# waiwera/waiwera

Measured on AMD Instinct MI355X. Metric: Newton steps/sec, 10M-cell eos_we (BCSR SpMV GB/s in roofline), higher is better.
Workload: dtype f64

## Files before the change

waiwera_amd/csrc/context.hpp:

```cpp
#pragma once
#include <hip/hip_runtime.h>
#include <string>
#include <type_traits>
#include <vector>
#include "../../include/waiwera_hip.h"
#include "devbuf.hpp"
#include "physics.hip.h"

namespace wai {

__host__ __device__ __forceinline__ size_t ell_ld(size_t n) {
  size_t ld = (n + 511) & ~(size_t)511;
  if ((ld & 262143) == 0) ld += 512;
  return ld;
}
__host__ __device__ __forceinline__ size_t ell_rows(int bs, size_t n) {
  if (bs >= 3) return ell_ld(n);
  return n;
}
__host__ __device__ __forceinline__ size_t ell_ix1(int bs, size_t n, int r, int k, size_t i) {
  if (bs >= 3) return ((i >> 6) * (size_t)(bs * bs) + (size_t)(r * bs + k)) * 64 + (i & 63);
  return ((size_t)r * n + i) * bs + k;
}
__host__ __device__ __forceinline__ size_t ell_ix(int bs, size_t n, int s, int r, int k, size_t i) {
// ... 40 lines not shown
  DevBuf<int> cell_src;
  DevBuf<int> face_cells;
};

struct Sources {
  int n = 0;
  DevBuf<int> cell, comp, next;
  DevBuf<double> rate, enth;
  DevBuf<SrcCtl> ctl;
  DevBuf<double> net;
};

struct NetNode { double rate = 0, enth = 0, wrate = 0, wenth = 0, srate = 0, senth = 0; };
struct NetRef { int kind = 0, index = -1; };
struct NetGroup {
  std::vector<NetRef> in;
  int scaling = 0;
  int n_limit = 0, limit_type[3] = {0, 0, 0};
  double limit[3] = {0, 0, 0};
  SrcCtl sep{};
  NetNode node;
};
struct NetOutput {
  int flow = 1;
  NetRef out;
  double rate = -1.0, proportion = -1.0, enthalpy = -1.0;
  NetNode node;
};
struct NetReinjector {
  NetRef in;
  std::vector<NetOutput> out;
  NetRef overflow;
  NetNode node;
  double in_w = 0, in_wh = 0, in_s = 0, in_sh = 0;
  double out_w = 0, out_s = 0;
  NetNode over;
  bool fed = false;
};
struct Network {
  bool on = false;
  std::vector<NetGroup> groups;
  std::vector<NetReinjector> reinjectors;
  std::vector<int> reinj_order;
  std::vector<int> rate_specified, enth_specified;
  std::vector<NetNode> src;
  std::vector<double> h_enth0, h_raw, out_rate, out_enth;
  std::vector<char> is_out;
  std::vector<SrcCtl> h_ctl;
  DevBuf<double> d_raw;
  std::vector<int> gidx;
  int n_global = 0;
  DevBuf<double> d_all;
  std::vector<double> h_loc, l_net, l_enth;
  std::vector<int> h_cell;
  bool coupling = true;
  bool cp_in_pc = true;
  bool cp_valid = false;
  std::vector<int> cp_cells;
  std::vector<double> h_cp_val;
  bool cp_span = false;
  int cp_m = 0, cp_j0 = 0;
  std::vector<int> cp_owner;
  DevBuf<int> d_cp_cells;
  DevBuf<double> d_cp_val, d_cp_f, d_cp_g;
  DevBuf<double> d_cp_x;
};

struct Bcsr {
  int n = 0, ncols = 0, nnzb = 0, bs = 0, W = 0;
  int* col = nullptr;
  double* val = nullptr;
  int* rowptr = nullptr;
  int dg = 0;
  double* fdg = nullptr;
};
struct Pattern {
  int n = 0, ncols = 0, nnzb = 0, W = 0;
  DevBuf<int> col;
  DevBuf<int> rowptr;
  std::vector<int> h_rowptr, h_colidx;
};

struct LinSys;
struct IluSchedule {
  int nsub = 0, max_rows = 0, max_lev = 0;
  DevBuf<int> sub_ptr;
  DevBuf<int> sub_nlev;
  DevBuf<int> sub_split;
  DevBuf<int> row_info;
  bool wide = false;
  DevBuf<unsigned long long> row_infow;
  DevBuf<double> fval;
  DevBuf<double> dinv;
  bool diag_only = false;
  bool scaled = true;
  bool park = true;
  DevBuf<int> row_uoff;
  DevBuf<int> row_tslot;
  int max_nl = 0;
  bool park2 = false;
  DevBuf<int> sub_int;
  DevBuf<int> sub_bnd;
  int n_int = 0, n_bnd = 0;
  DevBuf<int> sub_order;
  int max_ublocks = 0;
  bool fast3 = false;
  int max_nlu = 0;
  bool rows_kernel = false;
  bool wave_kernel = false;
  DevBuf<int> row_uoffw;
  int max_ublocks_w = 0;
  DevBuf<unsigned short> col16;
  DevBuf<int> sub_seg;
  bool level_sorted = false;
  bool big = false;
  bool sublu = false;
  int nlev_f = 0, nlev_b = 0;
  DevBuf<int> ord_f;
  DevBuf<int> ord_b;
  std::vector<int> lev_f_ptr, lev_b_ptr;
  bool built = false;
  const LinSys* owner = nullptr;
};
inline int pc_threads(const IluSchedule& s) { return ((s.max_rows + 63) / 64) * 64; }

template <class F>
int with_bs(int bs, F&& f) {
  switch (bs) {
    case 1: f(std::integral_constant<int, 1>{}); return 0;
    case 2: f(std::integral_constant<int, 2>{}); return 0;
    case 3: f(std::integral_constant<int, 3>{}); return 0;
    case 4: f(std::integral_constant<int, 4>{}); return 0;
    default: return -1;
  }
}
template <class F>
void with_flag(bool flag, F&& f) {
  if (flag) f(std::true_type{});
  else f(std::false_type{});
}
template <class F>
int with_eos(int kind, F&& f) {
  switch (kind) {
    case EOS_W: f(std::integral_constant<int, EOS_W>{}); return 0;
    case EOS_WE: f(std::integral_constant<int, EOS_WE>{}); return 0;
    case EOS_WCE: f(std::integral_constant<int, EOS_WCE>{}); return 0;
    case EOS_WSE: f(std::integral_constant<int, EOS_WSE>{}); return 0;
    case EOS_WAE: f(std::integral_constant<int, EOS_WAE>{}); return 0;
    case EOS_WSCE: f(std::integral_constant<int, EOS_WSCE>{}); return 0;
    case EOS_WSAE: f(std::integral_constant<int, EOS_WSAE>{}); return 0;
    default: return -1;
  }
}
struct EosTraits { int np, df, nmob; bool salt; };
inline int eos_traits(int kind, EosTraits& t) {
  return with_eos(kind, [&](auto k) {
    constexpr int K = decltype(k)::value;
    t = EosTraits{EosT<K>::np, EosT<K>::df, EosT<K>::nmob, is_salt<K>};
  });
}

struct AsmSystem {
  int overlap = -1;
  int levels = 0;
  bool sublu = false;
  int n_ext = 0;
  Bcsr E;
  DevBuf<int> E_col;
  DevBuf<double> E_val;
  IluSchedule sched;
  DevBuf<int> ext_row;
  DevBuf<int> gmap;
  DevBuf<double> r_ext;
  bool with_net = false;
  int n_net = 0;
  DevBuf<int> net_pos;
  DevBuf<int> net_pair;
  bool cross = false;
  DevBuf<double> hval;
  DevBuf<double> r_full;
};

struct ResForm {
  int method = 0;
  double dt = 0.0, ratio = 0.0;
  const double* last = nullptr;
  const double* last2 = nullptr;
};

constexpr int MAX_TRACERS = 8;
constexpr int POST_OFF = 64;
constexpr unsigned long long POST_KEY = 0x5bd1e995a5a5c3c3ull;
struct Tracers {
  int nt = 0;
  int phase[MAX_TRACERS] = {0};
  double decay[MAX_TRACERS] = {0}, activation[MAX_TRACERS] = {0}, diffusion[MAX_TRACERS] = {0};
// ... 245 lines not shown
```

waiwera_amd/csrc/kernels_fused.hip:

```cpp
#include "pc_generic.hip.h"
#include "pc_wide.hip.h"
#include "pc_park.hip.h"
#include "pc_rows.hip.h"
#include "pc_wave.hip.h"
#include "krylov_vec.hip.h"

namespace wai {

static inline int vgrid(int n) {
  int g = (n + TPB - 1) / TPB;
  return g > 1024 ? 1024 : (g < 1 ? 1 : g);
}

void read_env(wai_ctx* c) {
  c->env.fin_separate = getenv("WAI_FIN_SEPARATE") != nullptr;
  c->env.no_col16 = getenv("WAI_NO_COL16") != nullptr;
  c->env.scalar_kernels = getenv("WAI_BCGS_SCALAR_KERNELS") != nullptr;
}

int pc_kernel_kind(const wai_ctx* c, const Bcsr& J, const IluSchedule& s) {
  if (J.dg) return -1;
  if (s.wide) return 4;
  if (c->dbg) return 0;
  if (s.wave_kernel && J.bs >= 3) return 3;
  if (s.rows_kernel) return 2;
  if (J.bs == 2 && s.park && s.diag_only && s.scaled && s.fast3 && pc_threads(s) <= 512) return 1;
  return 0;
}
static bool kind_composes(int kind) { return kind >= 1 && kind <= 3; }
bool pc_axpy_capable(const wai_ctx* c, const Bcsr& M) { return !c->ilu.big && kind_composes(pc_kernel_kind(c, M, c->ilu)); }
bool pc_axpy_default(const wai_ctx* c, const Bcsr& M) {
  if (c->ilu.big) return false;
  const int kind = pc_kernel_kind(c, M, c->ilu);
  return (kind == 1 && c->ilu.col16 && !c->env.no_col16) || kind == 3;
}

template <int BS>
static void launch_pc_bs(wai_ctx* c, const Bcsr& J, const IluSchedule& s, bool spmv, const double* in, double* z,
                         int dot_mode, const double* aux, const int* list, int nrun, const Fin* finp, const double* in2) {
  if (!list) { nrun = s.nsub; list = s.sub_order; }
  const bool with_fin = finp && dot_mode != 0;
  Fin fin;
  if (finp && dot_mode != 0) { fin = *finp; fin.count = nrun; fin.nb = s.nsub; fin.nf = fin_slices(s.nsub); }
  c->ks.n_launch++;
  const int grid = ((nrun + 7) / 8) * 8 + (with_fin ? fin.nf : 0), T = pc_threads(s);
  const size_t lds = ((size_t)T * BS + 80) * sizeof(double);
  auto sp_ax = [&](auto&& go) {
    if (spmv) with_flag(in2 != nullptr, [&](auto ax) { go(std::true_type{}, ax); });
    else go(std::false_type{}, std::false_type{});
  };
  const int kind = pc_kernel_kind(c, J, s);
  const double* scal = c->ks.scal;
  const int* rp = (size_t)J.nnzb * 10 < (size_t)J.n * J.W * 9 ? J.rowptr : nullptr;
  if (kind == 4) {
    const size_t room = (size_t)64 * 1024 > lds ? (size_t)64 * 1024 - lds : 0;
    const int ucap = (int)std::min((size_t)s.max_ublocks_w, room / ((size_t)BS * BS * sizeof(double)));
    const size_t lds_w = lds + (size_t)ucap * BS * BS * sizeof(double);
    with_flag(spmv, [&](auto sp) {
      hipLaunchKernelGGL((k_pc_wide<BS, decltype(sp)::value>), grid, T, lds_w, c->stream, J.n, J.W, nrun, s.sub_ptr, s.sub_nlev,
                         s.row_infow, s.row_uoffw, J.col, rp, J.val, s.fval, in, z, aux, c->ks.partials, c->ks.nb_max,
                         dot_mode, ucap, list, fin);
    });
    return;
  }
  if (kind == 3) {
    if constexpr (BS >= 3) {
      const int ngrp = (nrun + 3) / 4;
      const int pbase = (list && list == s.sub_bnd) ? (s.n_int + 3) / 4 : 0, nb_w = pbase + ngrp;
      if (with_fin) { fin.nb = nb_w; fin.nf = fin_slices(nb_w); }
      c->ks.nb_pc = nb_w;
      const int gridw = ((ngrp + 7) / 8) * 8 + (with_fin ? fin.nf : 0);
      const int per = 64 * BS + s.max_ublocks_w * BS * BS;
      const size_t lds_w = (size_t)4 * per * sizeof(double);
      Stagger stagger;
      stagger.ncu = c->n_cu;
      stagger.per_cu = std::max(1, (int)((size_t)160 * 1024 / (lds_w + 864)));
      stagger.ticks = 400;
      sp_ax([&](auto sp, auto ax) {
        hipLaunchKernelGGL((k_pc_wave<BS, decltype(sp)::value, decltype(ax)::value>), gridw, 256, lds_w, c->stream, J.n, J.W, nrun,
                           s.sub_ptr, s.sub_nlev, s.row_info, s.row_uoffw, J.col, s.fval, s.dinv, in, in2, scal, z, aux, c->ks.partials,
                           c->ks.nb_max, dot_mode, list, rp, s.sub_split, per, pbase, fin, stagger);
      });
      return;
    }
  }
  if (kind == 2) {
    const int TR = ((s.max_rows * BS + 63) / 64) * 64;
    const size_t lds_r = ((size_t)s.max_rows * BS + BS + 5 * 16 + 8) * sizeof(double);
    auto rows = [&](auto nlu) {
      sp_ax([&](auto sp, auto ax) {
        constexpr int NLU = decltype(nlu)::value;
        hipLaunchKernelGGL((k_pc_rows<BS, decltype(sp)::value, NLU, NLU, decltype(ax)::value>), grid, TR, lds_r, c->stream, J.n, J.W,
                           nrun, s.sub_ptr, s.sub_nlev, s.row_info, J.col, s.fval, s.dinv, in, in2, scal, z, aux, c->ks.partials,
                           c->ks.nb_max, dot_mode, list, rp, s.sub_split, fin);
      });
    };
    if (s.max_nlu <= 3) rows(std::integral_constant<int, 3>{});
    else rows(std::integral_constant<int, 4>{});
    return;
  }
  if constexpr (BS == 2) {
    if (kind == 1) {
      const size_t lds_park = lds + (size_t)s.max_ublocks * 4 * sizeof(double);
      Stagger stagger;
      stagger.ncu = c->n_cu;
      stagger.per_cu = std::max(1, std::min(3, (int)((size_t)160 * 1024 / (lds_park + 704))));
      stagger.ticks = 600;
      with_flag(s.col16 && !c->env.no_col16, [&](auto c16) {
        sp_ax([&](auto sp, auto ax) {
          hipLaunchKernelGGL((k_pc_park<decltype(sp)::value, decltype(ax)::value, decltype(c16)::value>), grid, T, lds_park, c->stream,
                             J.n, J.W, nrun, s.sub_ptr, s.sub_nlev, s.row_info, s.row_uoff, J.col, s.col16, s.sub_seg, s.fval, s.dinv,
                             in, in2, scal, z, aux, c->ks.partials, c->ks.nb_max, dot_mode, list, fin, stagger);
        });
      });
      return;
    }
  }
  auto generic = [&](auto di) {
    with_flag(spmv, [&](auto sp) {
      with_flag(s.fast3, [&](auto fast) {
        hipLaunchKernelGGL((k_pc<BS, decltype(sp)::value, decltype(di)::value, decltype(fast)::value>), grid, T, lds, c->stream,
                           J.n, J.W, nrun, s.sub_ptr, s.sub_nlev, s.row_info, J.col, J.val, s.fval, s.dinv, in, z, aux,
                           c->ks.partials, c->ks.nb_max, dot_mode, c->dbg, list, fin);
      });
    });
  };
  if (s.diag_only && s.scaled) generic(std::integral_constant<int, 2>{});
  else if (s.diag_only) generic(std::integral_constant<int, 1>{});
  else generic(std::integral_constant<int, 0>{});
}

int launch_pc_on(wai_ctx* c, const Bcsr& M, const IluSchedule& s, bool spmv, const double* in, double* z,
                 int dot_mode, const double* aux, const int* list, int nrun, const Fin* fin, const double* in2) {
  if (in2 && (!spmv || !kind_composes(pc_kernel_kind(c, M, s)))) { c->err = "composed input asked of a kernel that cannot form it"; return -1; }
  const Fin* fin_later = nullptr;
  if (fin && dot_mode != 0 && c->env.fin_separate) { fin_later = fin; fin = nullptr; }
  if (M.dg) {
    c->ks.n_launch++;
    if (launch_dg_pc(c, M, s, spmv, in, z, list, nrun)) return -1;
    if (dot_mode == PC_DOT_NONE) return 0;
    const int n = M.dg * M.n, s0 = pc_dot_slot0(dot_mode);
    if (dot_mode == PC_DOT_ZA || dot_mode == PC_DOT_ZZ) vec_dots(c, z, dot_mode == PC_DOT_ZA ? aux : z, s0, nullptr, nullptr, 0, n);
    else {
      vec_dots(c, in, z, s0, z, z, s0 + 1, n);
      if (dot_mode == PC_DOT_MERGED) { vec_dots(c, in, in, s0 + 2, in, aux, s0 + 3, n); vec_dots(c, z, aux, s0 + 4, nullptr, nullptr, 0, n); }
    }
    if (const Fin* f = fin ? fin : fin_later) {
      if (dot_mode == PC_DOT_MERGED) { vec_finalize(c, c->ks.nb_pc, s0, 4, -1); vec_finalize(c, c->ks.nb_pc, s0 + 4, 1, f->phase); }
      else vec_finalize(c, c->ks.nb_pc, s0, pc_dot_nslots(dot_mode), f->phase);
      if (f->seq > 0) bcgs_post(c, f->seq);
    }
    return 0;
  }
  c->ks.nb_pc = s.nsub;
  if (with_bs(M.bs, [&](auto bs) { launch_pc_bs<decltype(bs)::value>(c, M, s, spmv, in, z, dot_mode, aux, list, nrun, fin, in2); }) != 0)
    return -1;
  if (fin_later) {
    vec_finalize(c, c->ks.nb_pc, fin_later->slot0, fin_later->nslots, fin_later->phase);
    if (fin_later->seq > 0) bcgs_post(c, fin_later->seq);
  }
  return 0;
}
int launch_pc(wai_ctx* c, const Bcsr& M, bool spmv, const double* in, double* z, int dot_mode, const double* aux,
              const int* list, int nrun, const Fin* fin, const double* in2) {
  return launch_pc_on(c, M, c->ilu, spmv, in, z, dot_mode, aux, list, nrun, fin, in2);
}
Fin make_fin(wai_ctx* c, int slot0, int nslots, int phase, bool post) {
  Fin f;
  f.slot0 = slot0; f.nslots = nslots; f.phase = phase;
  f.scal = c->ks.scal; f.post = c->ks.d_post; f.part2 = c->ks.partials2;
  f.seq = post ? ++c->ks.seq : 0;
  return f;
}

int vec_finalize(wai_ctx* c, int nb, int slot0, int nslots, int phase) {
  const int T = nb > 256 ? 1024 : 256;
  c->ks.n_launch++;
  hipLaunchKernelGGL(k_finalize, 1, T, 0, c->stream, c->ks.partials, c->ks.nb_max, nb, slot0, nslots, c->ks.scal, phase);
  return 0;
}

int vec_dot(wai_ctx* c, const double* a, const double* b, int n, int slot) {
  const int g = vgrid(n);
  c->ks.n_launch++;
  hipLaunchKernelGGL(k_dot, g, TPB, 0, c->stream, a, b, n, c->ks.partials, c->ks.nb_max, slot);
  return vec_finalize(c, g, slot, 1, -1);
}
int vec_dots(wai_ctx* c, const double* a1, const double* b1, int slot1, const double* a2, const double* b2,
             int slot2, int n) {
  const int g = vgrid(n);
  c->ks.n_launch++;
  hipLaunchKernelGGL(k_dots, g, TPB, 0, c->stream, a1, b1, slot1, a2, b2, slot2, n, c->ks.partials, c->ks.nb_max);
  c->ks.nb_pc = g;
  return 0;
// ... 137 lines not shown
```

waiwera_amd/csrc/measure.hip:

```cpp
#include "host.hpp"

using namespace wai;

namespace {
typedef double stream_d2 __attribute__((ext_vector_type(2)));
__global__ __launch_bounds__(256) void k_stream_copy(const stream_d2* __restrict__ src, stream_d2* __restrict__ dst, size_t n2) {
  const size_t stride = (size_t)gridDim.x * 256;
  size_t i = (size_t)blockIdx.x * 256 + threadIdx.x;
  for (; i + stride < n2; i += 2 * stride) {
    const stream_d2 a = __builtin_nontemporal_load(src + i), b = __builtin_nontemporal_load(src + i + stride);
    __builtin_nontemporal_store(a, dst + i);
    __builtin_nontemporal_store(b, dst + i + stride);
  }
  if (i < n2) __builtin_nontemporal_store(__builtin_nontemporal_load(src + i), dst + i);
}
__global__ __launch_bounds__(256) void k_stream_read(const stream_d2* __restrict__ src, size_t n2, double* sink) {
  const size_t stride = (size_t)gridDim.x * 256;
  size_t i = (size_t)blockIdx.x * 256 + threadIdx.x;
  double t = 0.0;
  for (; i + stride < n2; i += 2 * stride) {
    const stream_d2 a = __builtin_nontemporal_load(src + i), b = __builtin_nontemporal_load(src + i + stride);
    t += (a.x + a.y) + (b.x + b.y);
  }
  if (i < n2) { const stream_d2 a = __builtin_nontemporal_load(src + i); t += a.x + a.y; }
// ... 49 lines not shown
      case 19:
        hipLaunchKernelGGL(k_stream_copy, 8192, 256, 0, c->stream, reinterpret_cast<const stream_d2*>(c->flu_pert.get()),
                           reinterpret_cast<stream_d2*>(c->flu_pert + (copy_n & ~(size_t)1)), copy_n / 2);
        break;
      case 22:
        hipLaunchKernelGGL(k_stream_read, 8192, 256, 0, c->stream, reinterpret_cast<const stream_d2*>(c->flu_pert.get()), copy_n & ~(size_t)1,
                           c->ks.scal + 60);
        break;
      case 20: {
        const int m = std::min(std::max(sys.ksp.restart, 1), k.basis_m);
        for (int j = 0; j < m; j++) gmres_mdot(c, k.basis, (size_t)sys.nl, sys.n, k.T, j + 1);
        break;
      }
      case 21: {
        const int m = std::min(std::max(sys.ksp.restart, 1), k.basis_m);
        for (int j = 0; j < m; j++) gmres_maxpy_norm(c, k.basis, (size_t)sys.nl, sys.n, k.T, j + 1);
        break;
      }
      case 7:
        pc_amul(c, sys, k.R, k.T, PC_DOT_MERGED, k.RP, -1, pc_axpy_ok(c, sys) ? k.V : nullptr, false);
        break;
      case 11: pc_amul(c, sys, k.P, k.V, PC_DOT_NONE, nullptr, -2); break;
      case 12: pc_amul(c, sys, k.P, k.V, PC_DOT_ZA, k.RP, -2); break;
      case 13: pc_amul(c, sys, k.P, k.V, PC_DOT_XZ, nullptr, 3); break;
      case 14: pc_amul(c, sys, k.P, k.V, PC_DOT_MERGED, k.RP, -2); break;
      case 15: pc_amul(c, sys, k.P, k.V, PC_DOT_MERGED, k.RP, 6); break;
      default: pc_amul(c, sys, k.P, k.V, PC_DOT_ZA, k.RP, 2); break;
    }
  };
  c->dbg = (which == 3 || which == 4) && pc_fused(c, sys) && !(sys.A.bs == 2 && c->ilu.park) ? 1 : 0;
  partials_clear(c, S_D1, 5);
  if (c->comm && c->comm->nranks > 1) {
    for (int i = 0; i < 5; i++) run();
  } else {
    float warm = 0.f;
    int n = 0;
    HIPCHK(c, hipEventRecord(c->ev0, c->stream));
    do {
      for (int i = 0; i < 5; i++) run();
      n += 5;
      HIPCHK(c, hipEventRecord(c->ev1, c->stream));
      HIPCHK(c, hipEventSynchronize(c->ev1));
      HIPCHK(c, hipEventElapsedTime(&warm, c->ev0, c->ev1));
    } while (warm < 25.f && n < std::max(10, 2 * reps));
  }
  HIPCHK(c, hipEventRecord(c->ev0, c->stream));
  for (int i = 0; i < reps; i++) run();
  HIPCHK(c, hipEventRecord(c->ev1, c->stream));
  HIPCHK(c, hipEventSynchronize(c->ev1));
  c->dbg = 0;
  partials_clear(c, S_D1, 5);
  float ms = 0.f;
  HIPCHK(c, hipEventElapsedTime(&ms, c->ev0, c->ev1));
  *ms_per_launch = ms / reps;
  if (which == 20 || which == 21) *ms_per_launch /= (float)std::min(std::max(sys.ksp.restart, 1), k.basis_m);
  return 0;
}

const char* wai_pc_kernel_name(wai_ctx* c) {
  if (!c) return "";
  const IluSchedule& s = c->ilu;
  const LinSys& sys = c->flow;
  const int bs = sys.A.bs;
  const PcOpts pc = pc_of(c, sys);
  if (pc.type == WAI_PC_NONE) return "k_spmv (no preconditioner)";
  if (pc.type == WAI_PC_LU) return "k_spmv + k_lu_apply (dense block inverses)";
  static thread_local char buf[96];
  if (pc_sub_lu(pc)) {
    snprintf(buf, sizeof(buf), "k_spmv + k_sublu_solve on the extended system (%s, sub-preconditioner lu)",
             pc.type == WAI_PC_ASM ? "ASM" : "block Jacobi");
    return buf;
  }
  if (pc_extended(c, sys)) {
    snprintf(buf, sizeof(buf), "k_spmv + %s on the extended system (%s, ILU(%d))",
             sys.as.sched.big ? "k_lvl_solve per level" : (sys.as.sched.wide ? "k_pc_wide" : "k_pc"),
             pc.type == WAI_PC_ASM ? "ASM" : "block Jacobi", std::max(pc.ilu_levels, 0));
    return buf;
  }
  if (s.big) return "k_spmv + k_lvl_solve per level";
  switch (pc_kernel_kind(c, sys.A, s)) {
    case 4: snprintf(buf, sizeof(buf), "k_pc_wide<%d,spmv>", bs); break;
    case 3: snprintf(buf, sizeof(buf), "k_pc_wave<%d,spmv>", bs); break;
    case 2: snprintf(buf, sizeof(buf), "k_pc_rows<%d,spmv,%d+%d>", bs, s.max_nlu <= 3 ? 3 : 4, s.max_nlu <= 3 ? 3 : 4); break;
    case 1: return s.col16 && !getenv("WAI_NO_COL16") ? "k_pc_park<spmv,col16>" : "k_pc_park<spmv>";
    default:
      snprintf(buf, sizeof(buf), "k_pc<%d,spmv,%s,%s>", bs, s.diag_only ? (s.scaled ? "dilu-scaled" : "dilu") : "ilu",
               s.fast3 ? "compact3" : "generic");
  }
  return buf;
}
int wai_comm_size(wai_ctx* c) { return c ? comm_count(c->comm) : -2; }
int wai_bcgs_composed(wai_ctx* c) {
  if (!c) return -2;
  read_env(c);
  const BcgsPlan pl = bcgs_plan(c, c->flow);
  return pl.axpy ? 1 : 0;
}
int wai_launch_stats(wai_ctx* c, long long* kernels, long long* copies) {
  if (!c) return -2;
  if (kernels) *kernels = c->ks.n_launch;
  if (copies) *copies = c->ks.n_copy;
  return 0;
}
int wai_tracer_stats(wai_ctx* c, long long* assembly_sweeps) {
  if (!c) return -2;
  if (assembly_sweeps) *assembly_sweeps = c->tr.n_sweeps;
  return 0;
}
int wai_test_drop_partials(wai_ctx* c, int n) { return c ? test_drop_partials(c, n) : -2; }
int wai_test_device_memory(long long* allocations, long long* bytes) {
  if (!allocations || !bytes) return -2;
  *allocations = dev_live_allocs; *bytes = dev_live_bytes;
  return 0;
}
int wai_test_pc_operator(wai_ctx* c, int spmv, const double* x, const double* x2, double alpha, int dot_mode, const double* aux,
                         int split, int fin_phase, const double* scal_in, double* z, double* scal_out) {
  if (!c || !x || !z || !scal_in || !scal_out || dot_mode < PC_DOT_NONE || dot_mode > PC_DOT_MERGED || fin_phase < -2) return -2;
  if ((dot_mode == PC_DOT_ZA || dot_mode == PC_DOT_MERGED) && !aux) { c->err = "wai_test_pc_operator: dot modes 1 and 4 need aux"; return -2; }
  read_env(c);
  LinSys& sys = c->flow;
  if (c->ilu.owner != &sys) { const int e = do_pc_setup(c, sys); if (e) return e < 0 ? -1 : e; }
  if (x2 && (!spmv || !pc_operand_composable(c))) { c->err = "wai_test_pc_operator: composed operand asked of a kernel that cannot form it"; return -1; }
  if (split && (!spmv || !pc_fused(c, sys) || net_in_operator(c, sys) || c->ilu.n_int <= 0 || c->ilu.n_bnd <= 0 || !c->ilu.sub_int)) {
    c->err = "wai_test_pc_operator: no interior / face brick lists to split the launch over";
    return -1;
  }
  KrylovVecs& k = *sys.kv;
  const size_t n = (size_t)sys.n;
  double s[16];
  for (int i = 0; i < 16; i++) s[i] = scal_in[i];
  s[S_ALPHA] = alpha;
  HIPCHK(c, hipMemcpyAsync(k.R, x, n * sizeof(double), hipMemcpyDefault, c->stream));
  if (x2) HIPCHK(c, hipMemcpyAsync(k.V, x2, n * sizeof(double), hipMemcpyDefault, c->stream));
  if (aux) HIPCHK(c, hipMemcpyAsync(k.RP, aux, n * sizeof(double), hipMemcpyDefault, c->stream));
  HIPCHK(c, hipMemcpyAsync(c->ks.scal, s, sizeof(s), hipMemcpyHostToDevice, c->stream));
  partials_clear(c, S_D1, 5);
  const double* a = aux ? k.RP : nullptr;
  const double* v = x2 ? k.V : nullptr;
  int e = 0;
  if (split) {
    Fin fin;
    const Fin* fp = nullptr;
    if (fin_phase >= -1 && dot_mode) {
      fin = make_fin_dots(c, dot_mode, fin_phase);
      fp = &fin;
    }
    e = launch_pc_split(c, sys.A, k.R, k.T, dot_mode, a, fp, v, nullptr);
  } else if (spmv) {
    e = pc_amul(c, sys, k.R, k.T, dot_mode, a, fin_phase, v, false);
  } else {
    e = pc_solve(c, sys, k.R, k.T, dot_mode, k.R, a, fin_phase);
  }
  if (e) return e;
  if (fin_phase == -2 && dot_mode)
    vec_finalize(c, c->ks.nb_pc, pc_dot_slot0(dot_mode), pc_dot_nslots(dot_mode), -1);
  HIPCHK(c, hipMemcpyAsync(z, k.T, n * sizeof(double), hipMemcpyDefault, c->stream));
  HIPCHK(c, hipMemcpyAsync(s, c->ks.scal, sizeof(s), hipMemcpyDeviceToHost, c->stream));
  HIPCHK(c, hipStreamSynchronize(c->stream));
  for (int i = 0; i < 16; i++) scal_out[i] = s[i];
  return 0;
}
int wai_pc_axpy_capable(wai_ctx* c) { return c ? (pc_operand_composable(c) ? 1 : 0) : -2; }
int wai_test_drop_stream_wait(wai_ctx* c, int which) { if (!c) return -2; c->test_drop_wait = which; return 0; }
int wai_bench_mute_comm(wai_ctx* c, int on) {
  if (!c) return -2;
  if (c->comm) c->comm->mute = on != 0;
  return 0;
// ... 38 lines not shown
```

waiwera_amd/csrc/pc_park.hip.h:

```cpp
#pragma once
#include "reductions.hip.h"

namespace wai {

template <bool SPMV, bool AX, bool C16>
__global__ __launch_bounds__(512, 6) void k_pc_park(
    int n, int W, int nsub, const int* __restrict__ sub_ptr, const int* __restrict__ sub_nlev,
    const int* __restrict__ row_info, const int* __restrict__ row_uoff, const int* __restrict__ col,
    const unsigned short* __restrict__ col16, const int* __restrict__ sub_seg,
    const double* __restrict__ sval, const double* __restrict__ dinv, const double* __restrict__ in,
    const double* __restrict__ in2, const double* __restrict__ scal,
    double* __restrict__ z, const double* __restrict__ aux, double* partials, int nb_max, int dot,
    const int* __restrict__ sub_list, Fin fin, Stagger stagger) {
  constexpr int BS = 2, BB = 4, MLU = 3;
  extern __shared__ __attribute__((aligned(16))) double lds[];
  if (fin_block(fin, partials, nb_max)) return;
  int s = xcd_remap(blockIdx.x, nsub);
  if (s >= nsub) return;
  if (sub_list) s = sub_list[s];
  const int lo = sub_ptr[s], R = sub_ptr[s + 1] - lo;
  const int nl = sub_nlev[s];
  const int nlf = nl & 0xffff, nlb = nl >> 16;
  const int tid = threadIdx.x, i = lo + tid;
  const bool active = tid < R;
  const double nalpha = AX ? -scal[S_ALPHA] : 0.0;
  stagger_start(stagger);
  double* ys = lds;
  double* upark = lds + (size_t)blockDim.x * BS + 80;
  double Lf[MLU][BB];
  int Lc[MLU], Uc[MLU], lf = -1, lb = -1, uo = 0, nU = 0;
  double xin[BS] = {0.0, 0.0}, avp[BS] = {0.0, 0.0};
#pragma unroll
  for (int p = 0; p < MLU; p++) {
    Lc[p] = tid; Uc[p] = tid;
#pragma unroll
    for (int e = 0; e < BB; e++) Lf[p][e] = 0.0;
  }
  int lfirst = 0, dslot = 0, ulast = 0;
  int cgs[WMAX];
  if (active) {
    unpack_info(row_info[i], lfirst, dslot, ulast, lf, lb);
    uo = row_uoff[i];
    nU = ulast - dslot - 1;
    if constexpr (C16) {
      const int* sg = sub_seg + (size_t)s * 8;
      const int g0 = sg[0], g1 = sg[1], g2 = sg[2], g3 = sg[3], g4 = sg[4], g5 = sg[5], g6 = sg[6], g7 = sg[7];
      typedef unsigned wai_u4v __attribute__((ext_vector_type(4)));
      const wai_u4v pk = __builtin_nontemporal_load(reinterpret_cast<const wai_u4v*>(col16) + i);
      const unsigned pw[4] = {pk.x, pk.y, pk.z, pk.w};
      unsigned cu[WMAX];
#pragma unroll
      for (int q = 0; q < WMAX; q++) cu[q] = (pw[q >> 1] >> (16 * (q & 1))) & 0xffffu;
#pragma unroll
      for (int q = 0; q < WMAX; q++) {
        const unsigned code = cu[q] >> 13;
        int b = g0;
        b = code == 1 ? g1 : b; b = code == 2 ? g2 : b; b = code == 3 ? g3 : b; b = code == 4 ? g4 : b;
        b = code == 5 ? g5 : b; b = code == 6 ? g6 : b; b = code == 7 ? g7 : b;
        cgs[q] = q < W ? b + (int)(cu[q] & 8191u) : i;
      }
    } else {
#pragma unroll
      for (int q = 0; q < WMAX; q++) {
        cgs[q] = i;
        if (q < W) cgs[q] = load_col(col, (size_t)q * n + i);
      }
    }
  }
  double acc[BS] = {0.0, 0.0};
  if (active) {
#pragma unroll
    for (int q = 0; q < WMAX; q++) {
      if (q < W) {
        const int cg = cgs[q];
        double blk[BB];
        load_block<BS>(sval, n, q, i, blk);
        if constexpr (SPMV) {
          double xv[BS];
          load_xs<BS, AX>(in, in2, nalpha, cg, xv);
          acc[0] += blk[0] * xv[0] + blk[1] * xv[1];
          acc[1] += blk[2] * xv[0] + blk[3] * xv[1];
        }
        const bool isl = (q >= lfirst) && (q < dslot), isu = (q > dslot) && (q < ulast);
#pragma unroll
        for (int p = 0; p < MLU; p++) {
          const bool tl = isl && (q - lfirst == p), tu = isu && (q - dslot - 1 == p);
          Lc[p] = tl ? cg - lo : Lc[p];
          Uc[p] = tu ? cg - lo : Uc[p];
#pragma unroll
          for (int e = 0; e < BB; e++) Lf[p][e] = tl ? blk[e] : Lf[p][e];
        }
        if (isu) {
          double* dst = upark + (size_t)(uo + (q - dslot - 1)) * BB;
          *reinterpret_cast<double2*>(dst) = make_double2(blk[0], blk[1]);
          *reinterpret_cast<double2*>(dst + 2) = make_double2(blk[2], blk[3]);
        }
      }
    }
    if constexpr (!SPMV) {
      double r[BS], dv[BB];
      load_x<BS>(in, i, r);
      load_pivot<BS>(dinv, n, i, dv);
      acc[0] = dv[0] * r[0] + dv[1] * r[1];
      acc[1] = dv[2] * r[0] + dv[3] * r[1];
    }
    if (dot == PC_DOT_XZ || dot == PC_DOT_MERGED) load_xs<BS, AX>(in, in2, nalpha, i, xin);
    if (dot == PC_DOT_ZA || dot == PC_DOT_MERGED) load_x_stream<BS>(aux, i, avp);
  }
  if (active) *reinterpret_cast<double2*>(ys + tid * 2) = make_double2(acc[0], acc[1]);
  __syncthreads();
  auto gather3 = [&](const int (&cc)[MLU], const double (&ff)[MLU][BB], double* sum) {
    double2 yk[MLU];
#pragma unroll
    for (int p = 0; p < MLU; p++) yk[p] = *reinterpret_cast<const double2*>(ys + cc[p] * 2);
#pragma unroll
    for (int r = 0; r < BS; r++) {
      double part[MLU];
#pragma unroll
      for (int p = 0; p < MLU; p++) part[p] = ff[p][r * BS] * yk[p].x + ff[p][r * BS + 1] * yk[p].y;
      sum[r] = (part[0] + part[1]) + part[2];
    }
  };
  for (int lev = 1; lev < nlf; lev++) {
    if (lf == lev) {
      const double2 a = *reinterpret_cast<const double2*>(ys + tid * 2);
      double sum[BS];
      gather3(Lc, Lf, sum);
      *reinterpret_cast<double2*>(ys + tid * 2) = make_double2(a.x - sum[0], a.y - sum[1]);
    }
    __syncthreads();
  }
#pragma unroll
  for (int p = 0; p < MLU; p++) {
    const bool have = p < nU;
    const double* src = upark + (size_t)(uo + (have ? p : 0)) * BB;
    const double2 u0 = *reinterpret_cast<const double2*>(src), u1 = *reinterpret_cast<const double2*>(src + 2);
    Lf[p][0] = have ? u0.x : 0.0; Lf[p][1] = have ? u0.y : 0.0;
    Lf[p][2] = have ? u1.x : 0.0; Lf[p][3] = have ? u1.y : 0.0;
  }
  double out[BS] = {0.0, 0.0};
  for (int lev = 0; lev < nlb; lev++) {
    if (lb == lev) {
      const double2 a = *reinterpret_cast<const double2*>(ys + tid * 2);
      double sum[BS];
      gather3(Uc, Lf, sum);
      out[0] = a.x - sum[0];
      out[1] = a.y - sum[1];
      *reinterpret_cast<double2*>(ys + tid * 2) = make_double2(out[0], out[1]);
    }
    if (lev + 1 < nlb) __syncthreads();
  }
  if (active) store_z2(z, (size_t)i, out[0], out[1]);
  if (dot != 0) {
    double* red = lds + (size_t)blockDim.x * BS;
    double v[5] = {0.0, 0.0, 0.0, 0.0, 0.0};
    pc_row_dots<BS, true, false>(dot, v, out, active, [&](double (&x)[BS]) { x[0] = xin[0]; x[1] = xin[1]; },
                                 [&](double (&a)[BS]) { a[0] = avp[0]; a[1] = avp[1]; });
    __syncthreads();
    pc_reduce_dots(dot, v, red, partials, nb_max, s);
  }
}

}
```

waiwera_amd/csrc/pc_setup.hip:

```cpp
#include "host.hpp"

using namespace wai;

namespace wai {

int build_schedule(wai_ctx* c, IluSchedule& s, const std::vector<int>& rowptr, const std::vector<int>& colidx,
                   const std::vector<int>& sub, int N, int W, int np, bool ghosts, bool allow_wide, bool sublu) {
  s.nsub = (int)sub.size() - 1;
  if (sub.front() != 0 || sub.back() != N) { c->err = "sub_ptr must cover [0, n_owned]"; return -2; }
  std::vector<int> diag(N);
  for (int i = 0; i < N; i++) {
    const int* row = colidx.data() + rowptr[i];
    diag[i] = (int)(std::lower_bound(row, row + (rowptr[i + 1] - rowptr[i]), i) - row);
  }
  std::vector<int> info(N), uoff(N, 0), uoffw(N, 0), levf(N), levb(N), nlev(s.nsub, 0), lfirst(N), ulast(N), tslot(N, 0);
  int max_nu = 0;
  s.max_rows = 0; s.max_lev = 0; s.max_ublocks = 0; s.max_ublocks_w = 0; s.max_nlu = 0; s.max_nl = 0;
  bool offdiag_fill = false, fast3 = true;
  int nlf_all = 0, nlb_all = 0;
  for (int sd = 0; sd < s.nsub; sd++) {
    const int lo = sub[sd], hi = sub[sd + 1];
    if (hi < lo) { c->err = "sub_ptr not monotone"; return -2; }
    s.max_rows = std::max(s.max_rows, hi - lo);
    int nlf = 0, nlb = 0;
// ... 1 lines not shown
      const int* row = colidx.data() + rowptr[i];
      const int cnt = rowptr[i + 1] - rowptr[i];
      int ls = 0;
      while (ls < cnt && row[ls] < lo) ls++;
      int ue = cnt;
      while (ue > 0 && row[ue - 1] >= hi) ue--;
      lfirst[i] = ls; ulast[i] = ue;
      int lv = 0;
      for (int q = ls; q < diag[i]; q++) lv = std::max(lv, levf[row[q]] + 1);
      levf[i] = lv;
      nlf = std::max(nlf, lv + 1);
    }
    for (int i = hi - 1; i >= lo; i--) {
      const int* row = colidx.data() + rowptr[i];
      int lv = 0;
      for (int q = diag[i] + 1; q < ulast[i]; q++) lv = std::max(lv, levb[row[q]] + 1);
      levb[i] = lv;
      nlb = std::max(nlb, lv + 1);
    }
    for (int i = lo; i < hi && !offdiag_fill; i++) {
      const int* row = colidx.data() + rowptr[i];
      for (int q = lfirst[i]; q < diag[i] && !offdiag_fill; q++) {
        const int k = row[q];
        const int* rk = colidx.data() + rowptr[k];
        for (int r2 = diag[k] + 1; r2 < ulast[k]; r2++) {
          const int j = rk[r2];
          if (j == i) continue;
          if (std::binary_search(row + q + 1, row + ulast[i], j)) { offdiag_fill = true; break; }
        }
      }
    }
    for (int i = lo; i < hi; i++) {
      const int* row = colidx.data() + rowptr[i];
      int pack = 0;
      for (int q = lfirst[i], p = 0; q < diag[i] && p < 4; q++, p++) {
        const int k = row[q];
        const int* rk = colidx.data() + rowptr[k];
        const int* e = std::lower_bound(rk + diag[k] + 1, rk + ulast[k], i);
        const int r2 = (e < rk + ulast[k] && *e == i) ? (int)(e - rk) : 15;
        pack |= (r2 & 15) << (4 * p);
      }
      tslot[i] = pack;
      s.max_nl = std::max(s.max_nl, diag[i] - lfirst[i]);
    }
    int ucount = 0, ucountw = 0;
    for (int i = lo; i < hi; i++) {
      const int nL = diag[i] - lfirst[i], nU = ulast[i] - diag[i] - 1;
      if (nL > 3 || nU > 3 || lfirst[i] > 3 || diag[i] > 3) fast3 = false;
      s.max_nlu = std::max(s.max_nlu, std::max(nL, nU));
      uoff[i] = ucount;
      ucount += std::min(nU, 3);
      uoffw[i] = ucountw;
      ucountw += nU;
      max_nu = std::max(max_nu, nU);
    }
    s.max_ublocks = std::max(s.max_ublocks, ucount);
    s.max_ublocks_w = std::max(s.max_ublocks_w, ucountw);
    nlev[sd] = (nlf & 0xffff) | (nlb << 16);
    s.max_lev = std::max(s.max_lev, std::max(nlf, nlb));
    nlf_all = std::max(nlf_all, nlf); nlb_all = std::max(nlb_all, nlb);
  }
  s.sublu = sublu;
  s.wide = !sublu && allow_wide && c->pat.W > 8 && W > 8 && W <= 16 && s.max_rows <= 1024;
  s.big = sublu || s.max_rows > 1024 || (W > 8 && !s.wide);
  if (!s.big && s.max_lev > 1023) { c->err = "more than 1023 dependency levels in a subdomain"; return -2; }
  for (int i = 0; i < N; i++)
    info[i] = (s.big || s.wide) ? (lfirst[i] | (diag[i] << 8) | (ulast[i] << 16))
                                : (lfirst[i] | (diag[i] << 4) | (ulast[i] << 8) | (levf[i] << 12) | (levb[i] << 22));
  if (s.wide) {
    std::vector<unsigned long long> infow(N);
    for (int i = 0; i < N; i++)
      infow[i] = (unsigned long long)(lfirst[i] | (diag[i] << 5) | (ulast[i] << 10)) |
                 ((unsigned long long)(levf[i] | (levb[i] << 10)) << 32);
    if (s.row_infow.upload(c, infow)) return -1;
  }
  auto brick_cost = [&](int sd) { return ((nlev[sd] & 0xffff) + (nlev[sd] >> 16)) * 4096 + (sub[sd + 1] - sub[sd]); };
  auto lpt_order = [&](std::vector<int>& list) {
    const int n = (int)list.size(), per = (n + 7) >> 3;
    for (int j = 0; j < 8; j++) {
      const int a = std::min(j * per, n), b = std::min((j + 1) * per, n);
      std::stable_sort(list.begin() + a, list.begin() + b, [&](int x, int y) { return brick_cost(x) > brick_cost(y); });
    }
  };
  if (!s.big) {
    bool uniform = true;
    for (int sd = 1; sd < s.nsub && uniform; sd++) uniform = brick_cost(sd) == brick_cost(0);
    if (!uniform) {
      std::vector<int> order(s.nsub);
      std::iota(order.begin(), order.end(), 0);
      lpt_order(order);
      if (s.sub_order.upload(c, order)) return -1;
    }
  }
  if (ghosts) {
    std::vector<int> li, lb;
    for (int sd = 0; sd < s.nsub; sd++) {
      bool ghost = false;
      for (int i = sub[sd]; i < sub[sd + 1] && !ghost; i++)
        for (int q = rowptr[i]; q < rowptr[i + 1]; q++)
          if (colidx[q] >= N) { ghost = true; break; }
      (ghost ? lb : li).push_back(sd);
    }
    if (c->mesh.n_halo == 0 && W == 7) {
      li.clear(); lb.clear();
      for (int sd = 0; sd < s.nsub; sd++) {
        bool face = false;
        for (int i = sub[sd]; i < sub[sd + 1] && !face; i++) face = rowptr[i + 1] - rowptr[i] < 7;
        (face ? lb : li).push_back(sd);
      }
    }
    s.n_int = (int)li.size();
    s.n_bnd = (int)lb.size();
    lpt_order(li); lpt_order(lb);
    if (s.n_int > 0 && s.n_bnd > 0) {
      if (s.sub_int.upload(c, li) || s.sub_bnd.upload(c, lb)) return -1;
    }
  }
  if ((s.big || s.wide) && !sublu) {
    s.nlev_f = nlf_all; s.nlev_b = nlb_all;
    std::vector<int> of(N), ob(N);
    s.lev_f_ptr.assign(nlf_all + 1, 0); s.lev_b_ptr.assign(nlb_all + 1, 0);
    for (int i = 0; i < N; i++) { s.lev_f_ptr[levf[i] + 1]++; s.lev_b_ptr[levb[i] + 1]++; }
    for (int l = 0; l < nlf_all; l++) s.lev_f_ptr[l + 1] += s.lev_f_ptr[l];
    for (int l = 0; l < nlb_all; l++) s.lev_b_ptr[l + 1] += s.lev_b_ptr[l];
    std::vector<int> pf(s.lev_f_ptr.begin(), s.lev_f_ptr.end() - 1), pb(s.lev_b_ptr.begin(), s.lev_b_ptr.end() - 1);
    for (int i = 0; i < N; i++) { of[pf[levf[i]]++] = i; ob[pb[levb[i]]++] = i; }
    if (s.ord_f.upload(c, of) || s.ord_b.upload(c, ob)) return -1;
  }
  if (s.sub_ptr.upload(c, sub) || s.sub_nlev.upload(c, nlev) || s.row_info.upload(c, info) || s.row_uoff.upload(c, uoff) ||
      s.row_uoffw.upload(c, uoffw) || s.row_tslot.upload(c, tslot) || s.fval.alloc(c, ell_size(np, N, W)) ||
      s.dinv.alloc(c, (size_t)np * np * ell_rows(np, N)))
    return -1;
  s.diag_only = !offdiag_fill && !s.big && !s.wide;
  s.level_sorted = !s.big;
  for (int sd = 0; sd < s.nsub && s.level_sorted; sd++)
    for (int i = sub[sd] + 1; i < sub[sd + 1]; i++)
      if (levf[i] < levf[i - 1] || levb[i] > levb[i - 1]) { s.level_sorted = false; break; }
  s.fast3 = fast3;
  s.scaled = true;
#ifdef WAI_ILU_GENERAL
  s.diag_only = false;
#endif
  {
    const size_t need = ((size_t)(((s.max_rows + 63) / 64) * 64) * np + 32 + (size_t)s.max_ublocks * 4) * sizeof(double);
    s.park = need <= 64 * 1024;
  }
  {
    const bool can = s.diag_only && s.scaled && !s.big && s.max_nlu <= 4 && s.max_rows * np <= 1024 && W <= 8;
#ifdef WAI_PC_ROWS
    s.rows_kernel = can && (WAI_PC_ROWS != 0);
#else
    s.rows_kernel = can && np >= 3;
#endif
  }
  {
    const size_t lds_w = (size_t)4 * (64 * np + (size_t)s.max_ublocks_w * np * np) * sizeof(double);
    s.wave_kernel = s.rows_kernel && np == 3 && s.max_rows <= 64
                    && s.max_nl <= 3 && max_nu <= 4 && lds_w <= 64 * 1024;
#ifdef WAI_PC_WAVE
    s.wave_kernel = s.wave_kernel && (WAI_PC_WAVE != 0);
#endif
  }
  if (s.rows_kernel) {
    std::vector<int> split(s.nsub);
    bool any = false;
    for (int sd = 0; sd < s.nsub; sd++) {
      const int lo = sub[sd], hi = sub[sd + 1];
      int r1 = lo;
      while (r1 < hi && (rowptr[r1 + 1] - rowptr[r1]) * 2 > W) r1++;
      bool sorted = true;
      for (int i = r1; i < hi && sorted; i++) sorted = (rowptr[i + 1] - rowptr[i]) * 2 <= W;
      split[sd] = (sorted && r1 > lo) ? r1 - lo : hi - lo;
      any = any || split[sd] != hi - lo;
      int short_cnt = 0;
      for (int i = r1; i < hi; i++) short_cnt = std::max(short_cnt, rowptr[i + 1] - rowptr[i]);
      bool mixed = false;
      for (int i = lo; i < hi && !mixed; i++) mixed = (i < r1) != ((rowptr[i + 1] - rowptr[i]) * 2 > W);
      split[sd] |= (mixed || !sorted ? 15 : short_cnt) << 16;
    }
    if (any && s.sub_split.upload(c, split)) return -1;
  }
  if (np == 2 && W <= 8 && !s.big && s.park && s.diag_only && s.scaled && s.fast3 && s.max_rows <= 512) {
    std::vector<unsigned short> c16((size_t)8 * N, 0);
    std::vector<int> seg((size_t)s.nsub * 8, 0);
    std::vector<int> far;
    bool ok = true;
    int max_seg = 8;
    if (const char* e = getenv("WAI_COL16_MAX_SEG")) max_seg = std::max(1, std::min(8, atoi(e)));
    for (int sd = 0; sd < s.nsub && ok; sd++) {
      const int lo = sub[sd], hi = sub[sd + 1];
      far.clear();
      for (int i = lo; i < hi; i++)
        for (int q = rowptr[i]; q < rowptr[i + 1]; q++)
          if (colidx[q] < lo || colidx[q] >= hi) far.push_back(colidx[q]);
      std::sort(far.begin(), far.end());
      far.erase(std::unique(far.begin(), far.end()), far.end());
      int* sg = seg.data() + (size_t)sd * 8;
      int nseg = 1;
      sg[0] = lo;
      for (size_t k = 0; k < far.size();) {
        if (nseg == max_seg) { ok = false; break; }
        const int base = far[k];
        sg[nseg++] = base;
        while (k < far.size() && far[k] - base < 8192) k++;
      }
      for (int i = lo; i < hi && ok; i++) {
        const int cnt = rowptr[i + 1] - rowptr[i];
        for (int q = 0; q < W; q++) {
          const int cg = q < cnt ? colidx[rowptr[i] + q] : i;
          int sgi = 0;
          if (cg < lo || cg >= hi) {
            sgi = nseg - 1;
            while (sgi > 0 && !(cg >= sg[sgi] && cg - sg[sgi] < 8192)) sgi--;
            if (sgi == 0) { ok = false; break; }
          }
          c16[(size_t)i * 8 + q] = (unsigned short)((sgi << 13) | (cg - sg[sgi]));
        }
      }
    }
    if (ok && (s.col16.upload(c, c16) || s.sub_seg.upload(c, seg))) return -1;
  }
  s.built = true;
  return 0;
}

constexpr int ILU_COMPLETE_FILL = 1 << 28;
int iluk_fill(const std::vector<int>& ptr, int levels, int max_width, std::vector<int>& rp, std::vector<int>& col, std::vector<int>& src) {
  const int n = (int)rp.size() - 1;
  std::vector<int> orp(n + 1, 0), ocol, osrc, olev, odiag(n, 0);
  ocol.reserve(col.size() * (size_t)(1 + 2 * std::min(levels, 8))); osrc.reserve(ocol.capacity()); olev.reserve(ocol.capacity());
  std::vector<int> wc, wl, ws;
  for (size_t b = 0; b + 1 < ptr.size(); b++)
    for (int i = ptr[b]; i < ptr[b + 1]; i++) {
      wc.assign(col.begin() + rp[i], col.begin() + rp[i + 1]);
      ws.assign(src.begin() + rp[i], src.begin() + rp[i + 1]);
      wl.assign(wc.size(), 0);
      for (size_t a = 0; a < wc.size() && wc[a] < i; a++) {
        const int k = wc[a], lik = wl[a];
        for (int r = odiag[k] + 1; r < orp[k + 1]; r++) {
          const int j = ocol[r], lv = lik + olev[r] + 1;
          if (lv > levels) continue;
          const size_t pos = (size_t)(std::lower_bound(wc.begin() + a + 1, wc.end(), j) - wc.begin());
          if (pos < wc.size() && wc[pos] == j) { wl[pos] = std::min(wl[pos], lv); continue; }
          wc.insert(wc.begin() + pos, j); wl.insert(wl.begin() + pos, lv); ws.insert(ws.begin() + pos, -1);
        }
        if ((int)wc.size() > max_width) return (int)wc.size();
      }
      orp[i] = (int)ocol.size();
      odiag[i] = -1;
      for (size_t a = 0; a < wc.size(); a++) {
        if (wc[a] == i) odiag[i] = (int)ocol.size();
        ocol.push_back(wc[a]); osrc.push_back(ws[a]); olev.push_back(wl[a]);
      }
      orp[i + 1] = (int)ocol.size();
      if (odiag[i] < 0) odiag[i] = orp[i + 1] - 1;
    }
  rp.swap(orp); col.swap(ocol); src.swap(osrc);
  return 0;
}

int ensure_halo_dof(wai_ctx* c, int dof) {
  if (dof <= c->max_dof_buf) return 0;
  c->max_dof_buf = dof;
  return c->d_sendbuf.alloc(c, (size_t)c->send_total * dof) || c->d_recvbuf.alloc(c, (size_t)c->mesh.n_halo * dof) ? -1 : 0;
}

int ghost_rows(wai_ctx* c, const LinSys& sys, std::vector<int>& grp, std::vector<int>& gci, std::vector<int>& gslot) {
  const Pattern& J = c->pat;
  const int N = J.n, H = c->mesh.n_halo, W = J.W;
  std::vector<double> ids((size_t)N + H, -1.0);
  const double base = (double)c->comm->rank * 4294967296.0;
  for (int i = 0; i < N; i++) ids[i] = base + i;
  double* scratch = sys.kv->tmp;
  HIPCHK(c, hipMemcpyAsync(scratch, ids.data(), sizeof(double) * (N + H), hipMemcpyHostToDevice, c->stream));
  if (halo_exchange(c, scratch, 1)) return -1;
  HIPCHK(c, hipMemcpyAsync(ids.data(), scratch, sizeof(double) * (N + H), hipMemcpyDeviceToHost, c->stream));
  HIPCHK(c, hipStreamSynchronize(c->stream));
  if (ensure_halo_dof(c, W * sys.A.bs * sys.A.bs)) return -1;
  std::vector<int> sidx((size_t)c->send_total);
  HIPCHK(c, hipMemcpy(sidx.data(), c->d_send_idx, sizeof(int) * sidx.size(), hipMemcpyDeviceToHost));
  std::vector<double> sb((size_t)c->send_total * W, -1.0), rb((size_t)H * W, -1.0);
  for (int p = 0; p < c->send_total; p++) {
    const int i = sidx[p];
    for (int q = J.h_rowptr[i]; q < J.h_rowptr[i + 1]; q++) sb[(size_t)p * W + (q - J.h_rowptr[i])] = ids[J.h_colidx[q]];
  }
  HIPCHK(c, hipMemcpyAsync(c->d_sendbuf, sb.data(), sizeof(double) * sb.size(), hipMemcpyHostToDevice, c->stream));
  if (comm_exchange(c->comm, c->n_nbr, c->nbr_rank.data(), c->send_ptr.data(), c->recv_ptr.data(), W, c->d_sendbuf, c->d_recvbuf,
                    c->stream, c->err))
    return -1;
  HIPCHK(c, hipMemcpyAsync(rb.data(), c->d_recvbuf, sizeof(double) * rb.size(), hipMemcpyDeviceToHost, c->stream));
  HIPCHK(c, hipStreamSynchronize(c->stream));
  std::vector<std::pair<double, int>> known((size_t)N + H);
  for (int i = 0; i < N + H; i++) known[i] = {ids[i], i};
  std::sort(known.begin(), known.end());
  grp.assign((size_t)H + 1, 0);
  gci.clear(); gslot.clear();
  std::vector<std::pair<int, int>> row;
  for (int h = 0; h < H; h++) {
    row.clear();
    for (int q = 0; q < W; q++) {
      const double id = rb[(size_t)h * W + q];
      if (id < 0.0) continue;
      auto it = std::lower_bound(known.begin(), known.end(), std::make_pair(id, -1));
// ... 255 lines not shown
```

Measured before the change: 5.073.

## Pack park-kernel row metadata and per-subdomain brick records into aligned structs

Replaces the separate col16, row_info, row_uoff and sub_seg arrays with one 32-byte ParkRow record per row and one 64-byte ParkBrick record per subdomain, prebuilt for each launch list. Each row's compressed columns, info and U offset now arrive in two vector loads, and the subdomain bounds, level count and segment bases in one contiguous record, removing scattered indirections. In the AX path it also takes the diagonal x value from the SpMV loop instead of reloading it. This adds setup work and memory, and the compressed path is used only when the launch list matches one of the prebuilt brick lists.

Measured after the change: 4.989. -1.7%, worse.

```diff
diff --git a/waiwera_amd/csrc/context.hpp b/waiwera_amd/csrc/context.hpp
--- a/waiwera_amd/csrc/context.hpp
+++ b/waiwera_amd/csrc/context.hpp
@@ -146,6 +146,9 @@
 };
 
 struct LinSys;
+struct alignas(32) ParkRow { unsigned short col[8]; int info, uoff, pad[2]; };
+struct alignas(64) ParkBrick { int lo, hi, nlev, sub, seg[8], pad[4]; };
+static_assert(sizeof(ParkRow) == 32 && sizeof(ParkBrick) == 64, "one aligned record each");
 struct IluSchedule {
   int nsub = 0, max_rows = 0, max_lev = 0;
   DevBuf<int> sub_ptr;
@@ -174,8 +177,10 @@
   bool wave_kernel = false;
   DevBuf<int> row_uoffw;
   int max_ublocks_w = 0;
-  DevBuf<unsigned short> col16;
-  DevBuf<int> sub_seg;
+  DevBuf<ParkRow> park_rows;
+  DevBuf<ParkBrick> bricks_all;
+  DevBuf<ParkBrick> bricks_int;
+  DevBuf<ParkBrick> bricks_bnd;
   bool level_sorted = false;
   bool big = false;
   bool sublu = false;
diff --git a/waiwera_amd/csrc/kernels_fused.hip b/waiwera_amd/csrc/kernels_fused.hip
--- a/waiwera_amd/csrc/kernels_fused.hip
+++ b/waiwera_amd/csrc/kernels_fused.hip
@@ -32,7 +32,7 @@
 bool pc_axpy_default(const wai_ctx* c, const Bcsr& M) {
   if (c->ilu.big) return false;
   const int kind = pc_kernel_kind(c, M, c->ilu);
-  return (kind == 1 && c->ilu.col16 && !c->env.no_col16) || kind == 3;
+  return (kind == 1 && c->ilu.park_rows && !c->env.no_col16) || kind == 3;
 }
 
 template <int BS>
@@ -106,10 +106,12 @@
       stagger.ncu = c->n_cu;
       stagger.per_cu = std::max(1, std::min(3, (int)((size_t)160 * 1024 / (lds_park + 704))));
       stagger.ticks = 600;
-      with_flag(s.col16 && !c->env.no_col16, [&](auto c16) {
+      const ParkBrick* bricks = list == s.sub_order ? s.bricks_all.get() : list == s.sub_int ? s.bricks_int.get()
+                                : list == s.sub_bnd ? s.bricks_bnd.get() : nullptr;
+      with_flag(s.park_rows && bricks && !c->env.no_col16, [&](auto c16) {
         sp_ax([&](auto sp, auto ax) {
           hipLaunchKernelGGL((k_pc_park<decltype(sp)::value, decltype(ax)::value, decltype(c16)::value>), grid, T, lds_park, c->stream,
-                             J.n, J.W, nrun, s.sub_ptr, s.sub_nlev, s.row_info, s.row_uoff, J.col, s.col16, s.sub_seg, s.fval, s.dinv,
+                             J.n, J.W, nrun, s.sub_ptr, s.sub_nlev, s.row_info, s.row_uoff, J.col, s.park_rows, bricks, s.fval, s.dinv,
                              in, in2, scal, z, aux, c->ks.partials, c->ks.nb_max, dot_mode, list, fin, stagger);
         });
       });
diff --git a/waiwera_amd/csrc/measure.hip b/waiwera_amd/csrc/measure.hip
--- a/waiwera_amd/csrc/measure.hip
+++ b/waiwera_amd/csrc/measure.hip
@@ -155,7 +155,7 @@
     case 4: snprintf(buf, sizeof(buf), "k_pc_wide<%d,spmv>", bs); break;
     case 3: snprintf(buf, sizeof(buf), "k_pc_wave<%d,spmv>", bs); break;
     case 2: snprintf(buf, sizeof(buf), "k_pc_rows<%d,spmv,%d+%d>", bs, s.max_nlu <= 3 ? 3 : 4, s.max_nlu <= 3 ? 3 : 4); break;
-    case 1: return s.col16 && !getenv("WAI_NO_COL16") ? "k_pc_park<spmv,col16>" : "k_pc_park<spmv>";
+    case 1: return s.park_rows && !getenv("WAI_NO_COL16") ? "k_pc_park<spmv,col16>" : "k_pc_park<spmv>";
     default:
       snprintf(buf, sizeof(buf), "k_pc<%d,spmv,%s,%s>", bs, s.diag_only ? (s.scaled ? "dilu-scaled" : "dilu") : "ilu",
                s.fast3 ? "compact3" : "generic");
diff --git a/waiwera_amd/csrc/pc_park.hip.h b/waiwera_amd/csrc/pc_park.hip.h
--- a/waiwera_amd/csrc/pc_park.hip.h
+++ b/waiwera_amd/csrc/pc_park.hip.h
@@ -7,7 +7,7 @@
 __global__ __launch_bounds__(512, 6) void k_pc_park(
     int n, int W, int nsub, const int* __restrict__ sub_ptr, const int* __restrict__ sub_nlev,
     const int* __restrict__ row_info, const int* __restrict__ row_uoff, const int* __restrict__ col,
-    const unsigned short* __restrict__ col16, const int* __restrict__ sub_seg,
+    const ParkRow* __restrict__ rows, const ParkBrick* __restrict__ bricks,
     const double* __restrict__ sval, const double* __restrict__ dinv, const double* __restrict__ in,
     const double* __restrict__ in2, const double* __restrict__ scal,
     double* __restrict__ z, const double* __restrict__ aux, double* partials, int nb_max, int dot,
@@ -17,9 +17,18 @@
   if (fin_block(fin, partials, nb_max)) return;
   int s = xcd_remap(blockIdx.x, nsub);
   if (s >= nsub) return;
-  if (sub_list) s = sub_list[s];
-  const int lo = sub_ptr[s], R = sub_ptr[s + 1] - lo;
-  const int nl = sub_nlev[s];
+  int lo, R, nl, sg[8];
+  if constexpr (C16) {
+    const ParkBrick* __restrict__ b = bricks + s;
+    lo = b->lo; R = b->hi - lo; nl = b->nlev;
+#pragma unroll
+    for (int k = 0; k < 8; k++) sg[k] = b->seg[k];
+    s = b->sub;
+  } else {
+    if (sub_list) s = sub_list[s];
+    lo = sub_ptr[s]; R = sub_ptr[s + 1] - lo;
+    nl = sub_nlev[s];
+  }
   const int nlf = nl & 0xffff, nlb = nl >> 16;
   const int tid = threadIdx.x, i = lo + tid;
   const bool active = tid < R;
@@ -39,14 +48,22 @@
   int lfirst = 0, dslot = 0, ulast = 0;
   int cgs[WMAX];
   if (active) {
-    unpack_info(row_info[i], lfirst, dslot, ulast, lf, lb);
-    uo = row_uoff[i];
+    typedef unsigned wai_u4v __attribute__((ext_vector_type(4)));
+    typedef int wai_i2v __attribute__((ext_vector_type(2)));
+    wai_u4v pk;
+    if constexpr (C16) {
+      const ParkRow* __restrict__ r = rows + i;
+      pk = __builtin_nontemporal_load(reinterpret_cast<const wai_u4v*>(r));
+      const wai_i2v iu = __builtin_nontemporal_load(reinterpret_cast<const wai_i2v*>(r) + 2);
+      unpack_info(iu.x, lfirst, dslot, ulast, lf, lb);
+      uo = iu.y;
+    } else {
+      unpack_info(row_info[i], lfirst, dslot, ulast, lf, lb);
+      uo = row_uoff[i];
+    }
     nU = ulast - dslot - 1;
     if constexpr (C16) {
-      const int* sg = sub_seg + (size_t)s * 8;
       const int g0 = sg[0], g1 = sg[1], g2 = sg[2], g3 = sg[3], g4 = sg[4], g5 = sg[5], g6 = sg[6], g7 = sg[7];
-      typedef unsigned wai_u4v __attribute__((ext_vector_type(4)));
-      const wai_u4v pk = __builtin_nontemporal_load(reinterpret_cast<const wai_u4v*>(col16) + i);
       const unsigned pw[4] = {pk.x, pk.y, pk.z, pk.w};
       unsigned cu[WMAX];
 #pragma unroll
@@ -80,6 +97,10 @@
           load_xs<BS, AX>(in, in2, nalpha, cg, xv);
           acc[0] += blk[0] * xv[0] + blk[1] * xv[1];
           acc[1] += blk[2] * xv[0] + blk[3] * xv[1];
+          if constexpr (C16 && AX) {
+            xin[0] = q == dslot ? xv[0] : xin[0];
+            xin[1] = q == dslot ? xv[1] : xin[1];
+          }
         }
         const bool isl = (q >= lfirst) && (q < dslot), isu = (q > dslot) && (q < ulast);
 #pragma unroll
@@ -104,7 +125,8 @@
       acc[0] = dv[0] * r[0] + dv[1] * r[1];
       acc[1] = dv[2] * r[0] + dv[3] * r[1];
     }
-    if (dot == PC_DOT_XZ || dot == PC_DOT_MERGED) load_xs<BS, AX>(in, in2, nalpha, i, xin);
+    if constexpr (!(C16 && AX))
+      if (dot == PC_DOT_XZ || dot == PC_DOT_MERGED) load_xs<BS, AX>(in, in2, nalpha, i, xin);
     if (dot == PC_DOT_ZA || dot == PC_DOT_MERGED) load_x_stream<BS>(aux, i, avp);
   }
   if (active) *reinterpret_cast<double2*>(ys + tid * 2) = make_double2(acc[0], acc[1]);
diff --git a/waiwera_amd/csrc/pc_setup.hip b/waiwera_amd/csrc/pc_setup.hip
--- a/waiwera_amd/csrc/pc_setup.hip
+++ b/waiwera_amd/csrc/pc_setup.hip
@@ -107,18 +107,18 @@
       std::stable_sort(list.begin() + a, list.begin() + b, [&](int x, int y) { return brick_cost(x) > brick_cost(y); });
     }
   };
+  std::vector<int> order, li, lb;
   if (!s.big) {
     bool uniform = true;
     for (int sd = 1; sd < s.nsub && uniform; sd++) uniform = brick_cost(sd) == brick_cost(0);
     if (!uniform) {
-      std::vector<int> order(s.nsub);
+      order.resize(s.nsub);
       std::iota(order.begin(), order.end(), 0);
       lpt_order(order);
       if (s.sub_order.upload(c, order)) return -1;
     }
   }
   if (ghosts) {
-    std::vector<int> li, lb;
     for (int sd = 0; sd < s.nsub; sd++) {
       bool ghost = false;
       for (int i = sub[sd]; i < sub[sd + 1] && !ghost; i++)
@@ -206,7 +206,7 @@
     if (any && s.sub_split.upload(c, split)) return -1;
   }
   if (np == 2 && W <= 8 && !s.big && s.park && s.diag_only && s.scaled && s.fast3 && s.max_rows <= 512) {
-    std::vector<unsigned short> c16((size_t)8 * N, 0);
+    std::vector<ParkRow> rows((size_t)N, ParkRow{});
     std::vector<int> seg((size_t)s.nsub * 8, 0);
     std::vector<int> far;
     bool ok = true;
@@ -231,6 +231,9 @@
       }
       for (int i = lo; i < hi && ok; i++) {
         const int cnt = rowptr[i + 1] - rowptr[i];
+        if (diag[i] >= cnt || colidx[rowptr[i] + diag[i]] != i) { ok = false; break; }
+        rows[i].info = info[i];
+        rows[i].uoff = uoff[i];
         for (int q = 0; q < W; q++) {
           const int cg = q < cnt ? colidx[rowptr[i] + q] : i;
           int sgi = 0;
@@ -239,11 +242,26 @@
             while (sgi > 0 && !(cg >= sg[sgi] && cg - sg[sgi] < 8192)) sgi--;
             if (sgi == 0) { ok = false; break; }
           }
-          c16[(size_t)i * 8 + q] = (unsigned short)((sgi << 13) | (cg - sg[sgi]));
+          rows[i].col[q] = (unsigned short)((sgi << 13) | (cg - sg[sgi]));
         }
       }
     }
-    if (ok && (s.col16.upload(c, c16) || s.sub_seg.upload(c, seg))) return -1;
+    s.park_rows.reset(); s.bricks_all.reset(); s.bricks_int.reset(); s.bricks_bnd.reset();
+    if (ok) {
+      auto records = [&](const std::vector<int>* list, int count) {
+        std::vector<ParkBrick> b((size_t)count, ParkBrick{});
+        for (int p = 0; p < count; p++) {
+          const int sd = list ? (*list)[p] : p;
+          b[p].lo = sub[sd]; b[p].hi = sub[sd + 1]; b[p].nlev = nlev[sd]; b[p].sub = sd;
+          std::copy(seg.begin() + (size_t)sd * 8, seg.begin() + (size_t)sd * 8 + 8, b[p].seg);
+        }
+        return b;
+      };
+      if (s.park_rows.upload(c, rows) || s.bricks_all.upload(c, records(order.empty() ? nullptr : &order, s.nsub))) return -1;
+      if (!li.empty() && !lb.empty() &&
+          (s.bricks_int.upload(c, records(&li, (int)li.size())) || s.bricks_bnd.upload(c, records(&lb, (int)lb.size()))))
+        return -1;
+    }
   }
   s.built = true;
   return 0;
```
